# ToyotaResearchInstitute/idto

Measured on AMD Instinct MI355X. Metric: Gauss-Newton iters/sec (grad+Hessian+solve), mini_cheetah N=40, higher is better.
Workload: dtype f64; 1 GPU; mini_cheetah (nq=19, nv=18, 9 contact pairs), horizon N=40, dt=0.05, forward differences, one Gauss-Newton iteration per step; parallelism=single GPU

## Files before the change

### idto_amd/csrc/fd_kernel.h

```cpp
#pragma once

#include "arena_sizes.h"
#include "batch.h"
#include "id_eval.h"
#include "id_fast.h"

namespace idto_dev {

struct DevProblem {
  int N;
  double dt;
  const double* v_init;
  const double* q_nom;
  const double* v_nom;
  const double* Qq;
  const double* Qv;
  const double* R;
  const double* Qfq;
  const double* Qfv;
  const double* Qq0; const double* Qv0; const double* R0; const double* Qfq0; const double* Qfv0;
};

__host__ __device__ __forceinline__ DevProblem at_problem(DevProblem P, size_t o) {
  P.v_init = at_problem(P.v_init, o); P.q_nom = at_problem(P.q_nom, o); P.v_nom = at_problem(P.v_nom, o);
// ... 156 lines not shown
#pragma unroll
    for (int m = 0; m < NP; ++m) {
#pragma unroll
      for (int ur = 0; ur < TB; ++ur)
#pragma unroll
        for (int uc = 0; uc < TB; ++uc) {
          if (m == 0) acc[ur][uc] = a[m][ur].x * b[m][uc].x;
          else acc[ur][uc] = acc[ur][uc] + a[m][ur].x * b[m][uc].x;
          acc[ur][uc] = acc[ur][uc] + a[m][ur].y * b[m][uc].y;
        }
#pragma unroll
      for (int ur = 0; ur < TB; ++ur)
#pragma unroll
        for (int uc = 0; uc < TB; ++uc) asm volatile("" : "+v"(acc[ur][uc]));
      if (m == 0) FD_STAMP(18);
    }
    if (NV & 1) {
#pragma unroll
      for (int ur = 0; ur < TB; ++ur)
#pragma unroll
        for (int uc = 0; uc < TB; ++uc) acc[ur][uc] = acc[ur][uc] + A[ur][NV - 1] * B[uc][NV - 1];
    }
    FD_STAMP(19);
    return;
  }
  const int np = nv >> 1;
  double2 a[TB], b[TB];
#pragma unroll
  for (int u = 0; u < TB; ++u) {
    a[u] = reinterpret_cast<const double2*>(A[u])[0];
    b[u] = reinterpret_cast<const double2*>(B[u])[0];
  }
#pragma unroll
  for (int ur = 0; ur < TB; ++ur)
#pragma unroll
    for (int uc = 0; uc < TB; ++uc) {
      acc[ur][uc] = a[ur].x * b[uc].x;
      if (nv > 1) acc[ur][uc] = acc[ur][uc] + a[ur].y * b[uc].y;
    }
  FD_STAMP(18);
  double2 an[TB], bn[TB];
  if (np > 1) {
#pragma unroll
    for (int u = 0; u < TB; ++u) {
      an[u] = reinterpret_cast<const double2*>(A[u])[1];
      bn[u] = reinterpret_cast<const double2*>(B[u])[1];
    }
  }
  for (int m = 1; m < np; ++m) {
#pragma unroll
    for (int u = 0; u < TB; ++u) { a[u] = an[u]; b[u] = bn[u]; }
    const int mn = (m + 1 < np) ? m + 1 : m;
#pragma unroll
    for (int u = 0; u < TB; ++u) {
      an[u] = reinterpret_cast<const double2*>(A[u])[mn];
      bn[u] = reinterpret_cast<const double2*>(B[u])[mn];
    }
#pragma unroll
    for (int ur = 0; ur < TB; ++ur)
#pragma unroll
      for (int uc = 0; uc < TB; ++uc) {
        acc[ur][uc] = acc[ur][uc] + a[ur].x * b[uc].x;
        acc[ur][uc] = acc[ur][uc] + a[ur].y * b[uc].y;
      }
  }
  if ((nv & 1) && nv > 1) {
#pragma unroll
    for (int ur = 0; ur < TB; ++ur)
#pragma unroll
      for (int uc = 0; uc < TB; ++uc) acc[ur][uc] = acc[ur][uc] + A[ur][nv - 1] * B[uc][nv - 1];
  }
  FD_STAMP(19);
}


template <int SHAPE> struct FastShape {
  static constexpr TreeShape T = tree_shape(SHAPE);
  static constexpr int MAXC = T.MAXC, NP = T.NP, CJ = T.CJ, J0 = T.J0, K0 = T.K0, W2 = T.W2, GS = T.GS;
};
__host__ __device__ inline int fd_xch_doubles(int nxb, int threads, int npaths, int nstem = 0) {
  return (threads / npaths) * xch_eval_doubles(nxb, nstem);
}

template <int MAXC, int SHAPE = 0>
IDTO_DEV void fd_body(const DevModel& M, const DevContact& cp, const DevProblem& P, const double* __restrict__ q,
                      double* __restrict__ slab, int slab_stride, double* __restrict__ v_out,
                      double* __restrict__ a_out, double* __restrict__ nplus_out, const int k, int mode,
                      int stop_after, int echunk, double* __restrict__ terms) {
  extern __shared__ double lds[];
  constexpr bool FAST = SHAPE != 0 && SHAPE != SHAPE_XCH && SHAPE != SHAPE_STEM;
  const int tid = threadIdx.x, nt = blockDim.x;
  if (stop_after == 10) return;
#ifdef IDTO_FD_STAMPS
  long long st_arr[IDTO_FD_NSTAMPS] = {};
  long long* idto_fd_st = (tid == 0 || tid == IDTO_FD_STAMP_TID) ? st_arr : nullptr;
#endif
  FD_STAMP(0);
  const int nq = M.nq, nv = M.nv, K = M.npaths;
  const int bsz = nv * nq;
  const double dt = P.dt;

  const bool central = mode >= 2;
  const int NM = (mode == 2) ? 2 : ((mode == 3) ? 4 : 1);
  const int nP = (mode >= 1) ? NM * nq : 0;
  const int nT = (mode >= 1) ? NM * nq : 0;
  const int nM = (mode == 1) ? nv : (central ? NM * nq : 0);
  const int E = 1 + nP + nT + nM;

  double* qm1 = lds;
  double* q0 = qm1 + nq;
  double* q1 = q0 + nq;
  double* N0 = q1 + nq;
  double* N1 = N0 + bsz;
  double* v0 = N1 + bsz;
  double* v1 = v0 + nv;
  double* a0 = v1 + nv;
  double* edq = a0 + nv;
  const int EC = (echunk < E) ? echunk : E;
  double* edv = edq + E;
  double* eda = edv + E;
  double* etau = eda + E;
  double* eq = etau + E * nv;
  double* ev = eq + EC * nq;
  double* ea = ev + EC * nv;
  double* edump = ea + EC * nv;
  double* mblob = edump + nv;
  const int blob_lo = FAST ? M.fast_lo : 0, blob_n = FAST ? M.fast_n : M.blob_n;
  int* colinfo = reinterpret_cast<int*>(mblob + blob_n + (blob_n & 1));
  const int nvp = (nv + 1) & ~1, psz = nvp * nq;
  double* rec = reinterpret_cast<double*>(colinfo + nq + (nq & 1));
  rec += (rec - lds) & 1;
  double* xch = rec + (terms ? 6 * psz + 2 * nvp : 0);

  const bool sparse = M.nfloat == 0 || (M.nfloat > 0 && nt >= 128);
  const int ql = tid & 63, qcfg = tid >> 6;
  const bool quat_lane = sparse && M.nfloat > 0 && qcfg < 2 && ql >= 48 && ql < 60;
  double qf0[4];
  {
    const double* qq = q + (size_t)(k + (qcfg & 1)) * nq + (M.nfloat > 0 ? M.float_qs[0] : 0);
#pragma unroll
    for (int i = 0; i < 4; ++i) qf0[i] = qq[i];
  }
  double* wr = rec + 6 * psz;
  double* tw = wr + nvp;
  constexpr int BU = 8;
  double breg[BU];
#pragma unroll
  for (int u = 0; u < BU; ++u) {
    const int i = tid + u * nt;
    breg[u] = (i < blob_n) ? M.blob[blob_lo + i] : 0.0;
  }
  const bool qrow = tid < nq;
  const double g_qm1 = (qrow && k > 0) ? q[(k - 1) * nq + tid] : 0.0;
  const double g_q0 = qrow ? q[k * nq + tid] : 0.0, g_q1 = qrow ? q[(k + 1) * nq + tid] : 0.0;
  const double g_wr = (terms && mode != 0 && tid < nv) ? P.R[tid * nv + tid] : 0.0;
  const double g_nc0 = (sparse && tid < bsz) ? M.nplus_const[tid] : 0.0;
  const double g_nc1 = (sparse && tid + nt < bsz) ? M.nplus_const[tid + nt] : 0.0;
  const int g_ci = (sparse && qrow) ? M.colinfo[tid] : 0;
  const int rowinfo_r = (sparse && tid < nv) ? M.rowinfo[tid] : 0;
  asm volatile("" : "+v"(qf0[0]), "+v"(qf0[1]), "+v"(qf0[2]), "+v"(qf0[3]));
#pragma unroll
  for (int u = 0; u < BU; ++u) {
    const int i = tid + u * nt;
    if (i < blob_n) mblob[i] = breg[u];
  }
  for (int i = tid + BU * nt; i < blob_n; i += nt) mblob[i] = M.blob[blob_lo + i];
  if (qrow) { qm1[tid] = g_qm1; q0[tid] = g_q0; q1[tid] = g_q1; }
  for (int i = tid + nt; i < nq; i += nt) {
    qm1[i] = (k > 0) ? q[(k - 1) * nq + i] : 0.0;
    q0[i] = q[k * nq + i];
    q1[i] = q[(k + 1) * nq + i];
  }
  if (terms && mode != 0) {
    if (tid < nv) wr[tid] = g_wr;
    for (int l = tid + nt; l < nv; l += nt) wr[l] = P.R[l * nv + l];
  }
  if (sparse) {
    if (tid < bsz && g_nc0 == g_nc0) { N0[tid] = g_nc0; N1[tid] = g_nc0; }
    if (tid + nt < bsz && g_nc1 == g_nc1) { N0[tid + nt] = g_nc1; N1[tid + nt] = g_nc1; }
    for (int i = tid + 2 * nt; i < bsz; i += nt) {
      const double cst = M.nplus_const[i];
      if (cst == cst) { N0[i] = cst; N1[i] = cst; }
    }
    if (qrow) colinfo[tid] = g_ci;
    for (int i = tid + nt; i < nq; i += nt) colinfo[i] = M.colinfo[i];
    if (quat_lane) {
      const int e = ql - 48, r = e >> 2, c = e & 3;
      double* Nout = qcfg ? N1 : N0;
      for (int f = 0; f < M.nfloat; ++f) {
        const int qs = M.float_qs[f], vs = M.float_vs[f];
        double qq[4];
#pragma unroll
        for (int i = 0; i < 4; ++i) qq[i] = (f == 0) ? qf0[i] : q[(size_t)(k + qcfg) * nq + qs + i];
        const double nrm = __builtin_sqrt(((qq[0] * qq[0] + qq[1] * qq[1]) + qq[2] * qq[2]) + qq[3] * qq[3]);
        const double t0 = qq[0] / nrm, t1 = qq[1] / nrm, t2 = qq[2] / nrm, t3 = qq[3] / nrm;
        const double w2 = 2.0 * t0, x2 = 2.0 * t1, y2 = 2.0 * t2, z2 = 2.0 * t3;
        const double l0 = (r == 0) ? -x2 : ((r == 1) ? -y2 : -z2);
        const double l1 = (r == 0) ? w2 : ((r == 1) ? z2 : -y2);
        const double l2 = (r == 0) ? -z2 : ((r == 1) ? w2 : x2);
        const double l3 = (r == 0) ? y2 : ((r == 1) ? -x2 : w2);
        const double tc = (c == 0) ? t0 : ((c == 1) ? t1 : ((c == 2) ? t2 : t3));
        const double d0 = ((c == 0 ? 1.0 : 0.0) - t0 * tc) / nrm;
        const double d1 = ((c == 1 ? 1.0 : 0.0) - t1 * tc) / nrm;
        const double d2 = ((c == 2 ? 1.0 : 0.0) - t2 * tc) / nrm;
        const double d3 = ((c == 3 ? 1.0 : 0.0) - t3 * tc) / nrm;
        double acc = l0 * d0;
        acc += l1 * d1;
        acc += l2 * d2;
        acc += l3 * d3;
        Nout[(qs + c) * nv + vs + r] = acc;
      }
    }
  } else {
    for (int i = tid; i < bsz; i += nt) { N0[i] = 0.0; N1[i] = 0.0; }
  }
  FD_STAMP(1);
  __syncthreads();
  FD_STAMP(2);
  if (stop_after == 8) return;
  const DevModel Ml = rebase_model(M, mblob - blob_lo);
  if (!sparse) {
    for (int b = tid; b < Ml.nb; b += nt) {
      const int qs = Ml.qstart[b], vs = Ml.vstart[b], jt = Ml.jtype[b];
      if (jt == IDTO_JOINT_REVOLUTE || jt == IDTO_JOINT_PRISMATIC) colinfo[qs] = vs | 1 << 16;
      else if (jt == IDTO_JOINT_PLANAR) { for (int kq = 0; kq < 3; ++kq) colinfo[qs + kq] = (vs + kq) | 1 << 16; }
      else {
        for (int kq = 0; kq < 4; ++kq) colinfo[qs + kq] = vs | 3 << 16;
        for (int kq = 0; kq < 3; ++kq) colinfo[qs + 4 + kq] = (vs + 3 + kq) | 1 << 16;
      }
    }
    nplus_pair(Ml, q0, N0, q1, N1, tid, nt, true);
  }
  if (stop_after == 9) return;
  for (int r = tid; r < nv; r += nt) {
    double vr0, vr1;
    if (sparse) {
      const int ri = (r == tid) ? rowinfo_r : M.rowinfo[r];
      const int c0 = ri & 0xffff, c1 = c0 + (ri >> 16);
      double acc0 = N0[c0 * nv + r] * (q0[c0] - qm1[c0]), acc1 = N1[c0 * nv + r] * (q1[c0] - q0[c0]);
      for (int c = c0 + 1; c < c1; ++c) {
        acc0 += N0[c * nv + r] * (q0[c] - qm1[c]);
        acc1 += N1[c * nv + r] * (q1[c] - q0[c]);
      }
      vr0 = (k > 0) ? acc0 / dt : P.v_init[r];
      vr1 = acc1 / dt;
    } else {
      vr0 = (k > 0) ? velocity_row(Ml, N0, q0, qm1, dt, r) : P.v_init[r];
      vr1 = velocity_row(Ml, N1, q1, q0, dt, r);
    }
    v0[r] = vr0;
    v1[r] = vr1;
    a0[r] = (vr1 - vr0) / dt;
  }
  const double eps = 1.4901161193847656e-08;
  for (int e = (nt > 64) ? (tid + nt - 64) % nt : tid; e < E; e += nt) {
    double dq = 1.0;
    if (e >= 1 && (e < 1 + nP + nT || central)) {
      const int i = (e - 1) % nq;
      const double qi = (e < 1 + nP) ? q1[i] : ((e < 1 + nP + nT) ? q0[i] : qm1[i]);
      dq = eps * __builtin_fmax(1.0, __builtin_fabs(qi));
      const double temp = qi + dq;
      dq = temp - qi;
    }
    edq[e] = dq;
    const double dv = dq / dt;
    edv[e] = dv;
    eda[e] = dv / dt;
  }
  __syncthreads();

  auto trajectory_outputs = [&](int t0, int ts) {
    for (int r = t0; r < nv; r += ts) {
      v_out[(k + 1) * nv + r] = v1[r];
      a_out[k * nv + r] = a0[r];
      if (k == 0) v_out[r] = v0[r];
    }
    for (int i = t0; i < bsz; i += ts) {
      nplus_out[(size_t)(k + 1) * bsz + i] = N1[i];
      if (k == 0) nplus_out[i] = N0[i];
    }
  };
  const bool late_outputs = FAST && !central && stop_after != 1;
  if (!late_outputs) trajectory_outputs(tid, nt);

  FD_STAMP(3);
  if (stop_after == 1) return;
  const bool own_inputs = FAST && !central;
  for (int c0 = 0; c0 < E; c0 += (own_inputs ? E : EC)) {
  const int ce = own_inputs ? E : ((E - c0 < EC) ? E - c0 : EC);
  if (!own_inputs) {
  for (int idx = tid; idx < ce * nq; idx += nt) {
    const int el = idx / nq, c = idx - el * nq, e = c0 + el;
    double val = q1[c];
    if (e >= 1 && e < 1 + nP && c == (e - 1) % nq) {
      if (!central) {
        val = q1[c] + edq[e];
      } else {
        const int mi = (e - 1) / nq;
        const double mult = (mi == 0) ? 1.0 : ((mi == 1) ? -1.0 : ((mi == 2) ? 2.0 : -2.0));
        val = q1[c] + mult * edq[e];
      }
    }
    eq[idx] = val;
  }
  for (int idx = tid; idx < ce * nv; idx += nt) {
    const int el = idx / nv, j = idx - el * nv, e = c0 + el;
    double vv = v1[j], aa = a0[j];
    if (central && e >= 1) {
      const int g = (e - 1) / (NM * nq), mi = ((e - 1) / nq) % NM, i = (e - 1) % nq;
      const double mult = (mi == 0) ? 1.0 : ((mi == 1) ? -1.0 : ((mi == 2) ? 2.0 : -2.0));
      const double dv = edv[e], da = eda[e];
      const double n1 = N1[i * nv + j], n0 = N0[i * nv + j];
      if (g == 0) {
        vv = v1[j] + (mult * dv) * n1;
        aa = a0[j] + (mult * da) * n1;
      } else if (g == 1) {
        vv = v1[j] - (mult * dv) * n1;
        aa = a0[j] - (mult * da) * (n1 + n0);
      } else {
        aa = a0[j] + (mult * da) * n0;
      }
    } else if (e >= 1 && e < 1 + nP) {
      const int i = e - 1;
      const double dv = edv[e], da = eda[e];
      const double n1 = N1[i * nv + j];
      vv = v1[j] + dv * n1;
      aa = a0[j] + da * n1;
    } else if (e >= 1 + nP && e < 1 + nP + nT) {
      const int i = e - 1 - nP;
      const double dv = edv[e], da = eda[e];
      const double n1 = N1[i * nv + j], n0 = N0[i * nv + j];
      vv = v1[j] - dv * n1;
      aa = a0[j] - da * (n1 + n0);
    } else if (e >= 1 + nP + nT) {
      vv = 0.0;
      aa = (j == e - 1 - nP - nT) ? 1.0 : 0.0;
    }
    ev[idx] = vv;
    ea[idx] = aa;
  }
  __syncthreads();
  }

  if (stop_after == 2) return;
  const int groups = nt / K;
  if constexpr (FAST) {
    using FS = FastShape<SHAPE>;
    FastTab FT;
    FT.body = Ml.f_body; FT.cbody = Ml.f_cbody; FT.pairs = Ml.f_pairs; FT.seg = Ml.f_seg; FT.maxpp = Ml.f_maxpp;
    FT.gslots = Ml.gslots; FT.gcommon = Ml.gcommon;
    const int grp = tid / FS::NP, path = tid % FS::NP;
    for (int e0 = 0; e0 < ce; e0 += groups) {
      const int el = (e0 == 0) ? grp : e0 + (groups - 1 - grp);
      if (el < ce) {
        const bool full = central || c0 + el < 1 + nP + nT;
        if (own_inputs) {
          InFwd in;
          in.q1 = q1; in.v1 = v1; in.a0 = a0; in.N1 = N1; in.N0 = N0; in.nv = nv;
          in.kind = (el == 0) ? 0 : ((el < 1 + nP) ? 1 : ((el < 1 + nP + nT) ? 2 : 3));
          in.col = (el == 0) ? 0 : ((el < 1 + nP) ? el - 1 : ((el < 1 + nP + nT) ? el - 1 - nP : el - 1 - nP - nT));
          in.dq = edq[el];
          in.sdv = (in.kind == 2) ? -edv[el] : ((in.kind == 1) ? edv[el] : 0.0);
          in.sda = (in.kind == 2) ? -eda[el] : ((in.kind == 1) ? eda[el] : 0.0);
          in.keep = (in.kind == 3) ? 0ull : ~0ull;
          in.keep0 = (in.kind == 2) ? ~0ull : 0ull;
          id_eval_fast<FS::MAXC, FS::NP, FS::CJ, FS::J0, FS::K0, FS::W2, FS::GS>(FT, Ml.gravity, cp, path, full, in, etau + el * nv
#ifdef IDTO_FD_STAMPS
                                                                 , (e0 == 0) ? idto_fd_st : nullptr
#endif
          );
        } else {
          InLds in;
          in.q = eq + el * nq; in.v = ev + el * nv; in.a = ea + el * nv;
          id_eval_fast<FS::MAXC, FS::NP, FS::CJ, FS::J0, FS::K0, FS::W2, FS::GS>(FT, Ml.gravity, cp, path, full, in, etau + (c0 + el) * nv);
        }
      }
    }
    if (late_outputs && tid >= nt - 64) trajectory_outputs(tid - (nt - 64), 64);
  } else {
  for (int e0 = 0; e0 < ce; e0 += groups) {
    const int el = e0 + tid / K;
    const int path = tid % K;
    const int ee = (el < ce) ? el : 0;
    const bool full = central || c0 + ee < 1 + nP + nT;
    double* tau_dst = (el < ce) ? etau + (c0 + ee) * nv : edump;
    if constexpr (SHAPE == SHAPE_STEM)
      id_eval<MAXC, true, true>(Ml, cp, path, full, eq + ee * nq, ev + ee * nv, ea + ee * nv, tau_dst,
                                xch + (tid / K) * xch_eval_doubles(Ml.nxb, Ml.nstem));
    else if constexpr (SHAPE == SHAPE_XCH)
      id_eval<MAXC, true>(Ml, cp, path, full, eq + ee * nq, ev + ee * nv, ea + ee * nv, tau_dst, xch + (tid / K) * Ml.nxb * XREC);
    else
      id_eval<MAXC>(Ml, cp, path, full, eq + ee * nq, ev + ee * nv, ea + ee * nv, tau_dst);
  }
  }
  __syncthreads();
  }

  FD_STAMP(12);
  if (stop_after == 3) return;
  constexpr bool GROWS = FAST;
  constexpr bool CSIZES = FAST && SHAPE <= kNumSizedShapes;
  constexpr int CNQ = CSIZES ? tree_shape_nq(SHAPE) : 0, CNV = CSIZES ? tree_shape_nv(SHAPE) : 0, CNVP = (CNV + 1) & ~1;
  const int tnq = CNQ ? CNQ : nq, tnv = CNQ ? CNV : nv, tbsz = CNQ ? CNV * CNQ : bsz, tnvp = CNQ ? CNVP : nvp, tpsz = CNQ ? CNVP * CNQ : psz;
  double* sl = slab + (size_t)k * slab_stride;
  double* Mk = sl;
  double* Tk = sl + tbsz;
  double* Pk = sl + 2 * tbsz;
  double* tauk = sl + 3 * tbsz;
  for (int r = tid; r < tnv; r += nt) tauk[r] = etau[r];
  if constexpr (GROWS)
    if (terms && mode != 0)
      for (int r = nt - 1 - tid; r < tnvp; r += nt) tw[r] = (r < tnv) ? etau[r] * wr[r] : 0.0;
  if (mode == 1) {
    const double sc = 1 / dt / dt;
    const double* Mcols = etau + (1 + tnq + tnq) * tnv;
    const double fillM = (k == 0) ? __builtin_nan("") : 0.0;
    constexpr int RU = 2;
    for (int base = tid; base < tbsz; base += RU * nt) {
      int ii[RU], rr[RU], j0[RU], cnt[RU];
      bool ok[RU];
      double tp[RU], tt[RU], t0[RU], dqp[RU], dqt[RU], w[RU], mc[RU][3], n0[RU][3];
#pragma unroll
      for (int u = 0; u < RU; ++u) {
        const int idx = base + u * nt;
        ok[u] = idx < tbsz;
        const int id = ok[u] ? idx : 0;
        ii[u] = id / tnv; rr[u] = id - ii[u] * tnv;
        const int ci = colinfo[ii[u]];
        j0[u] = ci & 0xffff; cnt[u] = ci >> 16;
        tp[u] = etau[(1 + ii[u]) * tnv + rr[u]]; tt[u] = etau[(1 + tnq + ii[u]) * tnv + rr[u]]; t0[u] = etau[rr[u]];
        dqp[u] = edq[1 + ii[u]]; dqt[u] = edq[1 + tnq + ii[u]];
        w[u] = terms ? wr[rr[u]] : 0.0;
#pragma unroll
        for (int t = 0; t < 3; ++t) {
          const int j = (t < cnt[u]) ? j0[u] + t : j0[u];
          mc[u][t] = Mcols[j * tnv + rr[u]];
          n0[u][t] = N0[ii[u] * tnv + j];
        }
      }
      FD_STAMP(13);
      double pvs[RU], tvs[RU], accs[RU];
#pragma unroll
      for (int u = 0; u < RU; ++u) {
        if (!ok[u]) continue;
        pvs[u] = (tp[u] - t0[u]) / dqp[u];
        tvs[u] = (k >= 1) ? (tt[u] - t0[u]) / dqt[u] : 0.0;
        double acc = (sc * mc[u][0]) * n0[u][0];
        if (cnt[u] > 1) acc += (sc * mc[u][1]) * n0[u][1];
        if (cnt[u] > 2) acc += (sc * mc[u][2]) * n0[u][2];
// ... 56 lines not shown
  const float inb = 1.0f / (float)nb;
  for (int tile = tid; tile < ntiles; tile += nt) {
    if (stop_after == 6 && tile >= 3 * ntt) break;
    int xa, sb, tr, tc, ob;
    const bool lower = tile < 3 * ntt;
    if (lower) {
      const int which = (tile >= ntt) + (tile >= 2 * ntt);
      int rem = tile - which * ntt;
      tc = 0;
      if constexpr (CNQ != 0) {
        constexpr int NB = (CNQ + TB - 1) / TB, NBR = CNQ / TB + 1;
        int off = 0;
#pragma unroll
        for (int t = 0, S = 0; t < NB - 1; ++t) {
          S += NBR - t;
          const bool ge = rem >= S;
          tc += ge; off = ge ? S : off;
        }
        rem -= off;
      } else {
        while (rem >= nbr - tc) { rem -= nbr - tc; ++tc; }
      }
      tr = tc + rem;
      xa = which; sb = which; ob = which * qq;
    } else {
      const int it = tile - 3 * ntt, which = (it >= nbb) + (it >= 2 * nbb), e = it - which * nbb;
      if constexpr (CNQ != 0) tc = e / nb;
      else tc = (int)(((float)e + 0.5f) * inb);
      tr = e - tc * nb;
      xa = (which == 1) ? 1 : 0; sb = (which == 0) ? 1 : 2; ob = (3 + which) * qq;
    }
    const double* A[TB];
    const double* B[TB];
#pragma unroll
    for (int u = 0; u < TB; ++u) {
      const int r = tr * TB + u, c = tc * TB + u;
      if constexpr (GROWS) A[u] = r < tnq ? rec + (3 + xa) * tpsz + r * tnvp : tw;
      else A[u] = rec + (3 + xa) * tpsz + (r < tnq ? r : tnq - 1) * tnvp;
      B[u] = rec + sb * tpsz + (c < tnq ? c : tnq - 1) * tnvp;
    }
    double acc[TB][TB];
    FD_STAMP(17);
#ifdef IDTO_FD_STAMPS
    asm_dot_tile<TB, CNV>(A, B, tnv, acc, idto_fd_st);
#else
    asm_dot_tile<TB, CNV>(A, B, tnv, acc);
#endif
#pragma unroll
    for (int ur = 0; ur < TB; ++ur)
#pragma unroll
      for (int uc = 0; uc < TB; ++uc) {
        const int r = tr * TB + ur, c = tc * TB + uc;
        if (r < tnq && c < tnq && (!lower || r >= c)) stage[ob + c * tnq + r] = acc[ur][uc];
        if constexpr (GROWS)
          if (lower && r == tnq && c < tnq && stop_after != 7) stage[6 * qq + xa * tnq + c] = acc[ur][uc];
      }
    FD_STAMP(20);
  }
  FD_STAMP(21);
  if constexpr (!GROWS)
    if (stop_after != 7)
      for (int it = nt - 1 - tid; it < 3 * tnq; it += nt) {
        const int which = (it >= tnq) + (it >= 2 * tnq), j = it - which * tnq;
        const double* J = rec + which * tpsz + j * tnvp;
        double acc = (etau[0] * wr[0]) * J[0];
        for (int r = 1; r < tnv; ++r) acc += (etau[r] * wr[r]) * J[r];
        stage[6 * qq + which * tnq + j] = acc;
      }
  FD_STAMP(22);
#ifdef IDTO_FD_STAMPS
  if (idto_fd_st && k == 1 && 2 * IDTO_FD_NSTAMPS <= tbsz)
    for (int i = 0; i < IDTO_FD_NSTAMPS; ++i)
      nplus_out[(size_t)(k + 1) * tbsz + (tid == 0 ? 0 : IDTO_FD_NSTAMPS) + i] = (double)(st_arr[i] - st_arr[0]);
#endif
}

template <int MAXC, int SHAPE = 0>
__global__ void __launch_bounds__(256) fd_kernel(DevModel M, DevContact cp, DevProblem P, const double* __restrict__ q,
                          double* __restrict__ slab, int slab_stride, double* __restrict__ v_out,
                          double* __restrict__ a_out, double* __restrict__ nplus_out, int k_begin, int mode,
                          int stop_after, int echunk, size_t pstride, double* __restrict__ terms, AltSel alt) {
  const size_t o = (size_t)blockIdx.y * pstride;
  const size_t w = o + (size_t)alt_offset(alt, o);
  fd_body<MAXC, SHAPE>(M, cp, at_problem(P, o), at_problem(q, o), at_problem(slab, w), slab_stride, at_problem(v_out, w),
                       at_problem(a_out, w), at_problem(nplus_out, w), k_begin + (int)blockIdx.x, mode, stop_after, echunk,
                       terms ? at_problem(terms, w) : nullptr);
}

template <int MAXC, int SHAPE = 0>
__global__ void __launch_bounds__(256) fd_along_kernel(DevModel M, DevContact cp, DevProblem P, const double* __restrict__ q,
                          double* __restrict__ slab, int slab_stride, double* __restrict__ v_out,
                          double* __restrict__ a_out, double* __restrict__ nplus_out, int k_begin, int stop_after,
                          int echunk, size_t cstride, const double* __restrict__ gate) {
  if (gate && *gate != 0.0) return;
  const size_t w = (size_t)blockIdx.y * cstride;
  fd_body<MAXC, SHAPE>(M, cp, P, at_problem(q, w), at_problem(slab, w), slab_stride, at_problem(v_out, w),
                       at_problem(a_out, w), at_problem(nplus_out, w), k_begin + (int)blockIdx.x, 0, stop_after, echunk, nullptr);
}

template <int MAXC, int SHAPE = 0>
__global__ void __launch_bounds__(256) fd_along_batch_kernel(DevModel M, DevContact cp, DevProblem P, const double* __restrict__ q,
                          double* __restrict__ slab, int slab_stride, double* __restrict__ v_out,
                          double* __restrict__ a_out, double* __restrict__ nplus_out, int k_begin, int stop_after,
                          int echunk, size_t cstride, const double* __restrict__ gate, size_t pstride, size_t bstride,
                          size_t gstride) {
  if (gate && *at_problem(gate, (size_t)blockIdx.z * gstride) != 0.0) return;
  const size_t w = (size_t)blockIdx.z * bstride + (size_t)blockIdx.y * cstride;
  fd_body<MAXC, SHAPE>(M, cp, at_problem(P, (size_t)blockIdx.z * pstride), at_problem(q, w), at_problem(slab, w), slab_stride,
                       at_problem(v_out, w), at_problem(a_out, w), at_problem(nplus_out, w), k_begin + (int)blockIdx.x, 0,
                       stop_after, echunk, nullptr);
}

template <int MAXC, int SHAPE = 0>
__global__ void __launch_bounds__(256) fd_models_kernel(const double* __restrict__ records, size_t mstride, size_t cat, size_t mat,
                          DevProblem P, const double* __restrict__ q, double* __restrict__ slab, int slab_stride,
                          double* __restrict__ v_out, double* __restrict__ a_out, double* __restrict__ nplus_out, int k_begin,
                          int mode, int stop_after, int echunk, size_t pstride, double* __restrict__ terms, AltSel alt) {
  const size_t o = (size_t)blockIdx.y * pstride;
  const size_t w = o + (size_t)alt_offset(alt, o);
  const RecordPtr rec = record_at(records, (size_t)blockIdx.y * mstride);
  fd_body<MAXC, SHAPE>(*(const DevModel*)(rec + mat), *(const DevContact*)(rec + cat), at_problem(P, o), at_problem(q, o),
                       at_problem(slab, w), slab_stride, at_problem(v_out, w), at_problem(a_out, w), at_problem(nplus_out, w),
                       k_begin + (int)blockIdx.x, mode, stop_after, echunk, terms ? at_problem(terms, w) : nullptr);
}

template <int MAXC, int SHAPE = 0>
__global__ void __launch_bounds__(256) fd_along_models_kernel(const double* __restrict__ records, size_t mstride, size_t cat,
                          size_t mat, DevProblem P, const double* __restrict__ q, double* __restrict__ slab, int slab_stride,
                          double* __restrict__ v_out, double* __restrict__ a_out, double* __restrict__ nplus_out, int k_begin,
                          int stop_after, int echunk, size_t cstride, const double* __restrict__ gate, size_t pstride,
                          size_t bstride, size_t gstride) {
  if (gate && *at_problem(gate, (size_t)blockIdx.z * gstride) != 0.0) return;
  const size_t w = (size_t)blockIdx.z * bstride + (size_t)blockIdx.y * cstride;
  const RecordPtr rec = record_at(records, (size_t)blockIdx.z * mstride);
  fd_body<MAXC, SHAPE>(*(const DevModel*)(rec + mat), *(const DevContact*)(rec + cat), at_problem(P, (size_t)blockIdx.z * pstride),
                       at_problem(q, w), at_problem(slab, w), slab_stride, at_problem(v_out, w), at_problem(a_out, w),
                       at_problem(nplus_out, w), k_begin + (int)blockIdx.x, 0, stop_after, echunk, nullptr);
}

}
```

### idto_amd/csrc/id_fast.h

```cpp
#pragma once

#include "id_eval.h"

#ifdef IDTO_FD_STAMPS
#ifndef IDTO_FD_STAMP_TID
#define IDTO_FD_STAMP_TID 192
#endif
#define IDTO_FD_NSTAMPS 24
#define FD_STAMP(i) do { __builtin_amdgcn_sched_barrier(0); asm volatile("" ::: "memory"); if (idto_fd_st) idto_fd_st[i] = (long long)__builtin_readcyclecounter(); asm volatile("" ::: "memory"); __builtin_amdgcn_sched_barrier(0); } while (0)
#else
#define FD_STAMP(i) do { } while (0)
#endif

namespace idto_dev {

template <int CTRL>
IDTO_DEV double quad_perm(double x) {
  int lo = __double2loint(x), hi = __double2hiint(x);
  lo = __builtin_amdgcn_update_dpp(0, lo, CTRL, 0xf, 0xf, true);
  hi = __builtin_amdgcn_update_dpp(0, hi, CTRL, 0xf, 0xf, true);
  return __hiloint2double(hi, lo);
}
template <int NP>
IDTO_DEV V3 tree_sum_fast(V3 v) {
// ... 150 lines not shown
  const double exponent = -phi / cp.sigma;
  if (exponent >= 37) compliant_fn = -cp.k * phi;
  else compliant_fn = cp.sigma * cp.k * idto::detmath::log(1 + idto::detmath::exp(exponent));
  const double fn = compliant_fn * dissipation;
  const V3 that = (-vt) / __builtin_sqrt(cp.vs * cp.vs + dot(vt, vt));
  const V3 ft = (that * cp.mu) * fn;
  *fo = n1 * fn + ft;
  *fc = -*fo;
  *no = cross(pOC, *fo);
  *nc = cross(pCC, *fc);
  return true;
}

IDTO_DEV void inertial_wrench_rec(const double* rec, const M3& R, V3 w, V3 al, V3 a, V3 g, V3* f_in, V3* n_in) {
  const V3 cW = R * ldv3(rec + FB_COM);
  const V3 t1 = cross(al, cW);
  const V3 t2 = cross(w, cross(w, cW));
  const V3 acom = (a + t1) + t2;
  *f_in = (acom - g) * rec[FB_MASS];
  const V3 wB = tmul(R, w), alB = tmul(R, al);
  const double* I = rec + FB_INERTIA;
  const V3 Iw = mk(fma3(I[0], wB.x, I[3], wB.y, I[4], wB.z), fma3(I[3], wB.x, I[1], wB.y, I[5], wB.z),
                   fma3(I[4], wB.x, I[5], wB.y, I[2], wB.z));
  const V3 Ial = mk(fma3(I[0], alB.x, I[3], alB.y, I[4], alB.z), fma3(I[3], alB.x, I[1], alB.y, I[5], alB.z),
                    fma3(I[4], alB.x, I[5], alB.y, I[2], alB.z));
  const V3 nB = Ial + cross(wB, Iw);
  *n_in = R * nB + cross(cW, *f_in);
}

template <bool HAS_COMMON>
IDTO_DEV void pair_group(const double* plist, int segword, const DevContact& cp, const BodyState& C, const BodyState& cb,
                         V3* fext, V3* next, V3* cfe, V3* cne) {
  const int start = segword & 0xffff, count = segword >> 16;
  for (int j = start; j < start + count; ++j) {
    const double* pr = plist + j * FP_STRIDE;
    V3 fc, nc, fo, no;
    if (pair_eval<HAS_COMMON>(pr, cp, C, cb, &fc, &nc, &fo, &no)) {
      *fext = *fext + fc; *next = *next + nc;
      if (HAS_COMMON) {
        const bool oc = reinterpret_cast<const int*>(pr + FP_INFO)[3] != 0;
        if (oc) { *cfe = *cfe + fo; *cne = *cne + no; }
      }
    }
  }
}

struct FastTab {
  const double* body;
  const double* cbody;
  const double* pairs;
  const int* seg;
  int maxpp;
  unsigned long long gslots;
  int gcommon;
};

struct InLds {
  const double *q, *v, *a;
  IDTO_DEV double Q(int i) const { return q[i]; }
  IDTO_DEV double V(int j) const { return v[j]; }
  IDTO_DEV double A(int j) const { return a[j]; }
  IDTO_DEV InLds laundered() const { InLds o = *this; o.v = lds_launder(v); return o; }
};
struct InFwd {
  const double *q1, *v1, *a0, *N1, *N0;
  int nv, kind, col;
  double dq, sdv, sda;
  unsigned long long keep, keep0;
  IDTO_DEV static double and_bits(double x, unsigned long long m) {
    return __longlong_as_double((long long)((unsigned long long)__double_as_longlong(x) & m));
  }
  IDTO_DEV double Q(int i) const {
    const double x = q1[i], xp = x + dq;
    return (kind == 1 && i == col) ? xp : x;
  }
  IDTO_DEV double V(int j) const { return and_bits(v1[j], keep) + sdv * N1[col * nv + j]; }
  IDTO_DEV double A(int j) const {
    const double unit = (kind == 3 && j == col) ? 1.0 : 0.0;
    return (and_bits(a0[j], keep) + unit) + sda * (N1[col * nv + j] + and_bits(N0[col * nv + j], keep0));
  }
  IDTO_DEV InFwd laundered() const { InFwd o = *this; o.v1 = lds_launder(v1); o.N1 = lds_launder(N1); return o; }
};

template <int MAXC, int NP, int CJ, int J0, int K0, int W2, int GS = 0, class In>
IDTO_DEV void id_eval_fast(const FastTab& T, const double* gravity, const DevContact& cp, int path, bool full,
                           const In& in_fwd, double* tau, long long* idto_fd_st = nullptr) {
  const In& in = in_fwd;
  constexpr bool HAS_COMMON = (CJ == IDTO_JOINT_FLOATING);
  const V3 zero = mk(0, 0, 0);
  const V3 g = full ? mk(gravity[0], gravity[1], gravity[2]) : zero;
  const double* bt = T.body + (size_t)path * (MAXC * FB_STRIDE);
  const double* ct = T.cbody;
  const double* plist = T.pairs + (size_t)path * (T.maxpp * FP_STRIDE);
  const int* seg = T.seg + path * (MAXC + 2);

  int qs[MAXC], vs[MAXC];
#pragma unroll
  for (int s = 0; s < MAXC; ++s) {
    const int2 ix = *reinterpret_cast<const int2*>(bt + s * FB_STRIDE + FB_IDX);
    qs[s] = ix.x; vs[s] = ix.y;
  }
  int cqs = 0, cvs = 0;
  if (HAS_COMMON) {
    const int2 ix = *reinterpret_cast<const int2*>(ct + FB_IDX);
    cqs = ix.x; cvs = ix.y;
  }
  double qj[MAXC], vj[MAXC], aj[MAXC];
  double q0x = 0, q0y = 0, v0x = 0, v0y = 0, a0x = 0, a0y = 0;
#pragma unroll
  for (int s = 0; s < MAXC; ++s) {
    if (s == 0 && J0 == IDTO_JOINT_PLANAR) {
      q0x = in.Q(qs[0]); q0y = in.Q(qs[0] + 1); qj[0] = in.Q(qs[0] + 2);
      v0x = in.V(vs[0]); v0y = in.V(vs[0] + 1); vj[0] = in.V(vs[0] + 2);
      a0x = in.A(vs[0]); a0y = in.A(vs[0] + 1); aj[0] = in.A(vs[0] + 2);
    } else {
      qj[s] = in.Q(qs[s]); vj[s] = in.V(vs[s]); aj[s] = in.A(vs[s]);
    }
  }
  double cq[7], cv[6], ca[6];
  if (HAS_COMMON) {
#pragma unroll
    for (int i = 0; i < 7; ++i) cq[i] = in.Q(cqs + i);
#pragma unroll
    for (int i = 0; i < 6; ++i) { cv[i] = in.V(cvs + i); ca[i] = in.A(cvs + i); }
  }
  FD_STAMP(4);
  double sn[MAXC], cs[MAXC];
#pragma unroll
  for (int s = 0; s < MAXC; ++s) idto::detmath::sincos(qj[s], &sn[s], &cs[s]);
  FD_STAMP(5);

  double rc_next[FB_PREFETCH];
  prefetch_record(bt, rc_next);
  BodyState cb;
  cb.R = ident3(); cb.p = zero; cb.w = zero; cb.v = zero;
  V3 cb_al = zero, cb_a = zero, cb_fin = zero, cb_nin = zero;
  V3 cfe = zero, cne = zero;
  if (HAS_COMMON) {
    const M3 R_WF = ldm3(ct + FB_XPF);
    const V3 d1 = ldv3(ct + FB_XPF + 9);
    const M3 R_FM = quat_to_rot(cq);
    const V3 d2 = R_WF * mk(cq[4], cq[5], cq[6]);
    const V3 w_rel = R_WF * mk(cv[0], cv[1], cv[2]);
    const V3 v_rel = R_WF * mk(cv[3], cv[4], cv[5]);
    const V3 al_rel = R_WF * mk(ca[0], ca[1], ca[2]);
    const V3 a_rel = R_WF * mk(ca[3], ca[4], ca[5]);
    cb.R = R_WF * R_FM;
    cb.p = zero + (d1 + d2);
    cb.w = zero + w_rel;
    cb.v = zero + v_rel;
    cb_al = zero + al_rel;
    cb_a = zero + a_rel;
    inertial_wrench_rec(ct, cb.R, cb.w, cb_al, cb_a, GS ? body_gravity(T.gcommon != 0, g) : g, &cb_fin, &cb_nin);
    pin(cb_fin); pin(cb_nin);
    if (full) pair_group<false>(plist, seg[0], cp, cb, cb, &cfe, &cne, &cfe, &cne);
  }

  FD_STAMP(6);
  V3 r[MAXC], hW[MAXC], ft[MAXC], nt[MAXC];
  BodyState bs_prev;
  bs_prev.R = ident3(); bs_prev.p = zero; bs_prev.w = zero; bs_prev.v = zero;
  ParentKin P;
  P.R = ident3(); P.p = zero; P.w = zero; P.v = zero; P.al = zero; P.a = zero;
#pragma unroll
  for (int s = 0; s < MAXC; ++s) {
    double rec[FB_PREFETCH];
#pragma unroll
    for (int i = 0; i < FB_PREFETCH; ++i) rec[i] = rc_next[i];
    const bool world = (s == 0 && K0 == PK_WORLD) || (W2 >= 1 && s == W2);
    if (s == 0 && K0 == PK_COMMON) { P.R = cb.R; P.p = cb.p; P.w = cb.w; P.v = cb.v; P.al = cb_al; P.a = cb_a; }
    const M3 R_WF = world ? ldm3(rec + FB_XPF) : P.R * ldm3(rec + FB_XPF);
    const V3 d1 = world ? ldv3(rec + FB_XPF + 9) : P.R * ldv3(rec + FB_XPF + 9);
    BodyState bs;
    V3 al, acc;
    if (s == 0 && J0 == IDTO_JOINT_PLANAR) {
      M3 R_FM = ident3();
      R_FM.m[0] = cs[0]; R_FM.m[1] = -sn[0]; R_FM.m[3] = sn[0]; R_FM.m[4] = cs[0];
      const V3 ex = col(R_WF, 0), ey = col(R_WF, 1), ez = col(R_WF, 2);
      const V3 d2 = ex * q0x + ey * q0y;
      const V3 v_rel = ex * v0x + ey * v0y;
      const V3 a_rel = ex * a0x + ey * a0y;
      const V3 w_rel = ez * vj[0];
      const V3 al_rel = ez * aj[0];
      hW[0] = zero;
      bs.R = R_WF * R_FM;
      r[0] = d1 + d2;
      bs.p = zero + r[0];
      bs.w = zero + w_rel;
      bs.v = zero + v_rel;
      al = zero + al_rel;
      acc = zero + a_rel;
    } else {
      const V3 axis = ldv3(rec + FB_AXIS);
      const M3 R_FM = axis_angle(axis, sn[s], cs[s]);
      hW[s] = R_WF * axis;
      const V3 w_rel = hW[s] * vj[s];
      const V3 al_rel = hW[s] * aj[s];
      bs.R = R_WF * R_FM;
      r[s] = d1 + zero;
      if (world) {
        bs.p = zero + r[s];
        bs.w = zero + w_rel;
        bs.v = zero;
        al = zero + al_rel;
        acc = zero;
      } else {
        bs.p = P.p + r[s];
        bs.w = P.w + w_rel;
        bs.v = (P.v + cross(P.w, r[s])) + zero;
        al = (P.al + al_rel) + cross(P.w, w_rel);
        acc = ((P.a + cross(P.al, r[s])) + cross(P.w, cross(P.w, r[s]))) + zero;
      }
    }
    V3 fin, nin;
    inertial_wrench_rec(rec, bs.R, bs.w, al, acc, GS ? body_gravity(slot_gravity(T.gslots, path, s), g) : g, &fin, &nin);
    pin(fin); pin(nin); pin(r[s]); pin(hW[s]);
    if (s == MAXC - 1) FD_STAMP(8);
    if (s + 1 < MAXC) prefetch_record(bt + (s + 1) * FB_STRIDE, rc_next);
    V3 fext = zero, next = zero;
    if (W2 >= 1 && s == W2) {
      V3 ofe = zero, one = zero;
      if (full) pair_group<true>(plist, seg[1 + s], cp, bs, bs_prev, &fext, &next, &ofe, &one);
      ft[W2 - 1] = ft[W2 - 1] - ofe;
      nt[W2 - 1] = nt[W2 - 1] - one;
      pin(ft[W2 - 1]); pin(nt[W2 - 1]);
    } else if (full) {
      pair_group<HAS_COMMON>(plist, seg[1 + s], cp, bs, cb, &fext, &next, &cfe, &cne);
    }
    ft[s] = fin - fext;
    nt[s] = nin - next;
    pin(ft[s]); pin(nt[s]);
    if (W2 >= 1 && s == W2 - 1) bs_prev = bs;
    P.R = bs.R; P.p = bs.p; P.w = bs.w; P.v = bs.v; P.al = al; P.a = acc;
    if (s == 0) FD_STAMP(7);
    if (s == MAXC - 1) FD_STAMP(9);
  }
  if (HAS_COMMON && full) pair_group<false>(plist, seg[MAXC + 1], cp, cb, cb, &cfe, &cne, &cfe, &cne);

  FD_STAMP(10);
  const In inb = in_fwd.laundered();
  const double* btb = lds_launder(bt);
  V3 child_f = zero, child_n = zero;
  V3 root_f = zero, root_n = zero;
#pragma unroll
  for (int s = MAXC - 1; s >= 0; --s) {
    const double* rec = btb + s * FB_STRIDE;
    V3 f = ft[s], n = nt[s];
    if (s + 1 < MAXC && s + 1 != W2) { f = f + child_f; n = n + child_n; }
    if (s == 0 && J0 == IDTO_JOINT_PLANAR) {
      const M3 R_WF = ldm3(rec + FB_XPF);
      const double t0 = dot(col(R_WF, 0), f), t1 = dot(col(R_WF, 1), f), t2 = dot(col(R_WF, 2), n);
      tau[vs[0]] = full ? t0 + rec[FB_DAMP] * inb.V(vs[0]) : t0;
      tau[vs[0] + 1] = full ? t1 + rec[FB_DAMP + 1] * inb.V(vs[0] + 1) : t1;
      tau[vs[0] + 2] = full ? t2 + rec[FB_DAMP + 2] * inb.V(vs[0] + 2) : t2;
    } else {
      const double t = dot(hW[s], n);
      tau[vs[s]] = full ? t + rec[FB_DAMP] * inb.V(vs[s]) : t;
    }
    const V3 cf = f, cn = n + cross(r[s], f);
    if (s > 0) { child_f = cf; child_n = cn; }
    else if (K0 == PK_COMMON) { root_f = cf; root_n = cn; }
  }

  FD_STAMP(11);
  if (HAS_COMMON) {
    const V3 ext_f = tree_sum_fast<NP>(cfe);
    const V3 ext_n = tree_sum_fast<NP>(cne);
    const V3 ch_f = tree_sum_fast<NP>(root_f);
    const V3 ch_n = tree_sum_fast<NP>(root_n);
    const V3 f = (cb_fin - ext_f) + ch_f;
    const V3 n = (cb_nin - ext_n) + ch_n;
    if (path == 0) {
      const double* ctb = lds_launder(ct);
      const M3 R_WF = ldm3(ctb + FB_XPF);
      const V3 nF = tmul(R_WF, n), fF = tmul(R_WF, f);
      const double t6[6] = {nF.x, nF.y, nF.z, fF.x, fF.y, fF.z};
#pragma unroll
      for (int i = 0; i < 6; ++i) tau[cvs + i] = full ? t6[i] + ctb[FB_DAMP + i] * inb.V(cvs + i) : t6[i];
    }
  }
}

}
```

Baseline: 13250 GN iters/s.

## Precompute fast-ID front (indices, sincos) before barrier and reassign quaternion N+ to chain wave

Adds an AHEAD mode to the FD kernel. Non-chain waves compute the front part of the fast inverse dynamics (joint indices, configuration reads, sincos) for their first perturbation before the __syncthreads, so that work overlaps the velocity/acceleration setup. The last wave alone does the quaternion N+ entries and the v/a rows, using wave-level fences instead of a block barrier. Epsilon assignment is moved onto the remaining threads. This adds register pressure and more complex thread-role logic in exchange for shorter serialized latency per block.

```diff
diff --git a/idto_amd/csrc/fd_kernel.h b/idto_amd/csrc/fd_kernel.h
--- a/idto_amd/csrc/fd_kernel.h
+++ b/idto_amd/csrc/fd_kernel.h
@@ -262,7 +262,27 @@
   return (threads / npaths) * xch_eval_doubles(nxb, nstem);
 }
 
-template <int MAXC, int SHAPE = 0>
+IDTO_DEV double nplus_quat_entry(const double (&qq)[4], const int r, const int c) {
+  const double nrm = __builtin_sqrt(((qq[0] * qq[0] + qq[1] * qq[1]) + qq[2] * qq[2]) + qq[3] * qq[3]);
+  const double t0 = qq[0] / nrm, t1 = qq[1] / nrm, t2 = qq[2] / nrm, t3 = qq[3] / nrm;
+  const double w2 = 2.0 * t0, x2 = 2.0 * t1, y2 = 2.0 * t2, z2 = 2.0 * t3;
+  const double l0 = (r == 0) ? -x2 : ((r == 1) ? -y2 : -z2);
+  const double l1 = (r == 0) ? w2 : ((r == 1) ? z2 : -y2);
+  const double l2 = (r == 0) ? -z2 : ((r == 1) ? w2 : x2);
+  const double l3 = (r == 0) ? y2 : ((r == 1) ? -x2 : w2);
+  const double tc = (c == 0) ? t0 : ((c == 1) ? t1 : ((c == 2) ? t2 : t3));
+  const double d0 = ((c == 0 ? 1.0 : 0.0) - t0 * tc) / nrm;
+  const double d1 = ((c == 1 ? 1.0 : 0.0) - t1 * tc) / nrm;
+  const double d2 = ((c == 2 ? 1.0 : 0.0) - t2 * tc) / nrm;
+  const double d3 = ((c == 3 ? 1.0 : 0.0) - t3 * tc) / nrm;
+  double acc = l0 * d0;
+  acc += l1 * d1;
+  acc += l2 * d2;
+  acc += l3 * d3;
+  return acc;
+}
+
+template <int MAXC, int SHAPE = 0, bool AHEAD = false>
 IDTO_DEV void fd_body(const DevModel& M, const DevContact& cp, const DevProblem& P, const double* __restrict__ q,
                       double* __restrict__ slab, int slab_stride, double* __restrict__ v_out,
                       double* __restrict__ a_out, double* __restrict__ nplus_out, const int k, int mode,
@@ -314,10 +334,21 @@
 
   const bool sparse = M.nfloat == 0 || (M.nfloat > 0 && nt >= 128);
   const int ql = tid & 63, qcfg = tid >> 6;
-  const bool quat_lane = sparse && M.nfloat > 0 && qcfg < 2 && ql >= 48 && ql < 60;
+  constexpr bool FRONT = AHEAD && FAST && SHAPE <= kNumSizedShapes && tree_shape(FAST ? SHAPE : 1).CJ == IDTO_JOINT_FLOATING;
+  bool front = false, chain_wave = false;
+  int qsel = qcfg & 1, vrow = tid;
+  if constexpr (FRONT) {
+    front = mode == 1 && sparse && M.nfloat == 1 && stop_after != 1;
+    if (front) {
+      chain_wave = __builtin_amdgcn_readfirstlane(qcfg) == (nt >> 6) - 1;
+      qsel = (ql >= 12 && ql < 24) ? 1 : 0;
+      vrow = chain_wave ? ql : nv;
+    }
+  }
+  const bool quat_lane = sparse && M.nfloat > 0 && qcfg < 2 && ql >= 48 && ql < 60 && !front;
   double qf0[4];
   {
-    const double* qq = q + (size_t)(k + (qcfg & 1)) * nq + (M.nfloat > 0 ? M.float_qs[0] : 0);
+    const double* qq = q + (size_t)(k + qsel) * nq + (M.nfloat > 0 ? M.float_qs[0] : 0);
 #pragma unroll
     for (int i = 0; i < 4; ++i) qf0[i] = qq[i];
   }
@@ -337,7 +368,7 @@
   const double g_nc0 = (sparse && tid < bsz) ? M.nplus_const[tid] : 0.0;
   const double g_nc1 = (sparse && tid + nt < bsz) ? M.nplus_const[tid + nt] : 0.0;
   const int g_ci = (sparse && qrow) ? M.colinfo[tid] : 0;
-  const int rowinfo_r = (sparse && tid < nv) ? M.rowinfo[tid] : 0;
+  const int rowinfo_r = (sparse && vrow < nv) ? M.rowinfo[vrow] : 0;
   asm volatile("" : "+v"(qf0[0]), "+v"(qf0[1]), "+v"(qf0[2]), "+v"(qf0[3]));
 #pragma unroll
   for (int u = 0; u < BU; ++u) {
@@ -372,23 +403,7 @@
         double qq[4];
 #pragma unroll
         for (int i = 0; i < 4; ++i) qq[i] = (f == 0) ? qf0[i] : q[(size_t)(k + qcfg) * nq + qs + i];
-        const double nrm = __builtin_sqrt(((qq[0] * qq[0] + qq[1] * qq[1]) + qq[2] * qq[2]) + qq[3] * qq[3]);
-        const double t0 = qq[0] / nrm, t1 = qq[1] / nrm, t2 = qq[2] / nrm, t3 = qq[3] / nrm;
-        const double w2 = 2.0 * t0, x2 = 2.0 * t1, y2 = 2.0 * t2, z2 = 2.0 * t3;
-        const double l0 = (r == 0) ? -x2 : ((r == 1) ? -y2 : -z2);
-        const double l1 = (r == 0) ? w2 : ((r == 1) ? z2 : -y2);
-        const double l2 = (r == 0) ? -z2 : ((r == 1) ? w2 : x2);
-        const double l3 = (r == 0) ? y2 : ((r == 1) ? -x2 : w2);
-        const double tc = (c == 0) ? t0 : ((c == 1) ? t1 : ((c == 2) ? t2 : t3));
-        const double d0 = ((c == 0 ? 1.0 : 0.0) - t0 * tc) / nrm;
-        const double d1 = ((c == 1 ? 1.0 : 0.0) - t1 * tc) / nrm;
-        const double d2 = ((c == 2 ? 1.0 : 0.0) - t2 * tc) / nrm;
-        const double d3 = ((c == 3 ? 1.0 : 0.0) - t3 * tc) / nrm;
-        double acc = l0 * d0;
-        acc += l1 * d1;
-        acc += l2 * d2;
-        acc += l3 * d3;
-        Nout[(qs + c) * nv + vs + r] = acc;
+        Nout[(qs + c) * nv + vs + r] = nplus_quat_entry(qq, r, c);
       }
     }
   } else {
@@ -412,10 +427,20 @@
     nplus_pair(Ml, q0, N0, q1, N1, tid, nt, true);
   }
   if (stop_after == 9) return;
-  for (int r = tid; r < nv; r += nt) {
+  if constexpr (FRONT)
+    if (chain_wave) {
+      if (ql < 24) {
+        const int e = (ql < 12) ? ql : ql - 12, r = e >> 2, c = e & 3;
+        (qsel ? N1 : N0)[(M.float_qs[0] + c) * nv + M.float_vs[0] + r] = nplus_quat_entry(qf0, r, c);
+      }
+      __builtin_amdgcn_fence(__ATOMIC_RELEASE, "wavefront");
+      __builtin_amdgcn_wave_barrier();
+      __builtin_amdgcn_fence(__ATOMIC_ACQUIRE, "wavefront");
+    }
+  for (int r = vrow; r < nv; r += (front ? 64 : nt)) {
     double vr0, vr1;
     if (sparse) {
-      const int ri = (r == tid) ? rowinfo_r : M.rowinfo[r];
+      const int ri = (r == vrow) ? rowinfo_r : M.rowinfo[r];
       const int c0 = ri & 0xffff, c1 = c0 + (ri >> 16);
       double acc0 = N0[c0 * nv + r] * (q0[c0] - qm1[c0]), acc1 = N1[c0 * nv + r] * (q1[c0] - q0[c0]);
       for (int c = c0 + 1; c < c1; ++c) {
@@ -433,7 +458,8 @@
     a0[r] = (vr1 - vr0) / dt;
   }
   const double eps = 1.4901161193847656e-08;
-  for (int e = (nt > 64) ? (tid + nt - 64) % nt : tid; e < E; e += nt) {
+  const int elo = (front && nt >= 192) ? 64 : 0, ew = (front && nt > 64) ? nt - 64 - elo : nt;
+  for (int e = front ? ((tid >= elo && tid < elo + ew) ? tid - elo : E) : ((nt > 64) ? (tid + nt - 64) % nt : tid); e < E; e += ew) {
     double dq = 1.0;
     if (e >= 1 && (e < 1 + nP + nT || central)) {
       const int i = (e - 1) % nq;
@@ -447,6 +473,27 @@
     edv[e] = dv;
     eda[e] = dv / dt;
   }
+  using FS = FastShape<FAST ? SHAPE : 1>;
+  FastFront<FS::MAXC> pre;
+  const bool formed = front && !chain_wave;
+  if constexpr (FRONT)
+    if (formed) {
+      const int el = tid / FS::NP;
+      if (el < E) {
+        FastTab FT;
+        FT.body = Ml.f_body; FT.cbody = Ml.f_cbody;
+        InFwd in;
+        in.q1 = q1; in.v1 = v1; in.a0 = a0; in.N1 = N1; in.N0 = N0; in.nv = nv;
+        in.kind = (el >= 1 && el < 1 + nP) ? 1 : 0;
+        in.col = (in.kind == 1) ? el - 1 : 0;
+        const double qi = q1[in.col];
+        double dq = eps * __builtin_fmax(1.0, __builtin_fabs(qi));
+        const double temp = qi + dq;
+        in.dq = temp - qi;
+        id_fast_front<FS::MAXC, FS::CJ, FS::J0>(FT, tid % FS::NP, in, pre);
+      }
+      FD_STAMP(23);
+    }
   __syncthreads();
 
   auto trajectory_outputs = [&](int t0, int ts) {
@@ -525,7 +572,6 @@
   if (stop_after == 2) return;
   const int groups = nt / K;
   if constexpr (FAST) {
-    using FS = FastShape<SHAPE>;
     FastTab FT;
     FT.body = Ml.f_body; FT.cbody = Ml.f_cbody; FT.pairs = Ml.f_pairs; FT.seg = Ml.f_seg; FT.maxpp = Ml.f_maxpp;
     FT.gslots = Ml.gslots; FT.gcommon = Ml.gcommon;
@@ -540,11 +586,14 @@
           in.kind = (el == 0) ? 0 : ((el < 1 + nP) ? 1 : ((el < 1 + nP + nT) ? 2 : 3));
           in.col = (el == 0) ? 0 : ((el < 1 + nP) ? el - 1 : ((el < 1 + nP + nT) ? el - 1 - nP : el - 1 - nP - nT));
           in.dq = edq[el];
+          if constexpr (FRONT)
+            if (!(formed && e0 == 0)) id_fast_front<FS::MAXC, FS::CJ, FS::J0>(FT, path, in, pre);
           in.sdv = (in.kind == 2) ? -edv[el] : ((in.kind == 1) ? edv[el] : 0.0);
           in.sda = (in.kind == 2) ? -eda[el] : ((in.kind == 1) ? eda[el] : 0.0);
           in.keep = (in.kind == 3) ? 0ull : ~0ull;
           in.keep0 = (in.kind == 2) ? ~0ull : 0ull;
-          id_eval_fast<FS::MAXC, FS::NP, FS::CJ, FS::J0, FS::K0, FS::W2, FS::GS>(FT, Ml.gravity, cp, path, full, in, etau + el * nv
+          id_eval_fast<FS::MAXC, FS::NP, FS::CJ, FS::J0, FS::K0, FS::W2, FS::GS>(FT, Ml.gravity, cp, path, full, in, pre,
+                                                                 FRONT, etau + el * nv
 #ifdef IDTO_FD_STAMPS
                                                                  , (e0 == 0) ? idto_fd_st : nullptr
 #endif
@@ -767,9 +816,9 @@
                           int stop_after, int echunk, size_t pstride, double* __restrict__ terms, AltSel alt) {
   const size_t o = (size_t)blockIdx.y * pstride;
   const size_t w = o + (size_t)alt_offset(alt, o);
-  fd_body<MAXC, SHAPE>(M, cp, at_problem(P, o), at_problem(q, o), at_problem(slab, w), slab_stride, at_problem(v_out, w),
-                       at_problem(a_out, w), at_problem(nplus_out, w), k_begin + (int)blockIdx.x, mode, stop_after, echunk,
-                       terms ? at_problem(terms, w) : nullptr);
+  fd_body<MAXC, SHAPE, true>(M, cp, at_problem(P, o), at_problem(q, o), at_problem(slab, w), slab_stride, at_problem(v_out, w),
+                             at_problem(a_out, w), at_problem(nplus_out, w), k_begin + (int)blockIdx.x, mode, stop_after, echunk,
+                             terms ? at_problem(terms, w) : nullptr);
 }
 
 template <int MAXC, int SHAPE = 0>
diff --git a/idto_amd/csrc/id_fast.h b/idto_amd/csrc/id_fast.h
--- a/idto_amd/csrc/id_fast.h
+++ b/idto_amd/csrc/id_fast.h
@@ -256,9 +256,54 @@
   IDTO_DEV InFwd laundered() const { InFwd o = *this; o.v1 = lds_launder(v1); o.N1 = lds_launder(N1); return o; }
 };
 
+template <int MAXC>
+struct FastFront {
+  int qs[MAXC], vs[MAXC], cqs, cvs;
+  double q0x, q0y, cq[7], sn[MAXC], cs[MAXC];
+};
+template <int MAXC, int CJ, int J0, class In>
+IDTO_DEV void id_fast_front(const FastTab& T, int path, const In& in, FastFront<MAXC>& F) {
+  constexpr bool HAS_COMMON = (CJ == IDTO_JOINT_FLOATING);
+  const double* bt = T.body + (size_t)path * (MAXC * FB_STRIDE);
+  const double* ct = T.cbody;
+#pragma unroll
+  for (int s = 0; s < MAXC; ++s) {
+    const int2 ix = *reinterpret_cast<const int2*>(bt + s * FB_STRIDE + FB_IDX);
+    F.qs[s] = ix.x; F.vs[s] = ix.y;
+  }
+  F.cqs = 0; F.cvs = 0;
+  if (HAS_COMMON) {
+    const int2 ix = *reinterpret_cast<const int2*>(ct + FB_IDX);
+    F.cqs = ix.x; F.cvs = ix.y;
+  }
+  double qj[MAXC];
+  F.q0x = 0; F.q0y = 0;
+#pragma unroll
+  for (int s = 0; s < MAXC; ++s) {
+    if (s == 0 && J0 == IDTO_JOINT_PLANAR) {
+      F.q0x = in.Q(F.qs[0]); F.q0y = in.Q(F.qs[0] + 1); qj[0] = in.Q(F.qs[0] + 2);
+    } else {
+      qj[s] = in.Q(F.qs[s]);
+    }
+  }
+#pragma unroll
+  for (int i = 0; i < 7; ++i) F.cq[i] = HAS_COMMON ? in.Q(F.cqs + i) : 0.0;
+#pragma unroll
+  for (int s = 0; s < MAXC; ++s) idto::detmath::sincos(qj[s], &F.sn[s], &F.cs[s]);
+#pragma unroll
+  for (int s = 0; s < MAXC; ++s) asm volatile("" : "+v"(F.qs[s]), "+v"(F.vs[s]), "+v"(F.sn[s]), "+v"(F.cs[s]));
+  if (HAS_COMMON) {
+    asm volatile("" : "+v"(F.cqs), "+v"(F.cvs));
+#pragma unroll
+    for (int i = 0; i < 7; ++i) asm volatile("" : "+v"(F.cq[i]));
+  }
+  if (J0 == IDTO_JOINT_PLANAR) asm volatile("" : "+v"(F.q0x), "+v"(F.q0y));
+}
+
 template <int MAXC, int NP, int CJ, int J0, int K0, int W2, int GS = 0, class In>
 IDTO_DEV void id_eval_fast(const FastTab& T, const double* gravity, const DevContact& cp, int path, bool full,
-                           const In& in_fwd, double* tau, long long* idto_fd_st = nullptr) {
+                           const In& in_fwd, const FastFront<MAXC>& pre, bool have_pre, double* tau,
+                           long long* idto_fd_st = nullptr) {
   const In& in = in_fwd;
   constexpr bool HAS_COMMON = (CJ == IDTO_JOINT_FLOATING);
   const V3 zero = mk(0, 0, 0);
@@ -269,18 +314,42 @@
   const int* seg = T.seg + path * (MAXC + 2);
 
   int qs[MAXC], vs[MAXC];
+  int cqs = 0, cvs = 0;
+  double qj[MAXC], vj[MAXC], aj[MAXC];
+  double q0x = 0, q0y = 0, v0x = 0, v0y = 0, a0x = 0, a0y = 0;
+  double cq[7], cv[6], ca[6];
+  double sn[MAXC], cs[MAXC];
+  if (have_pre) {
+#pragma unroll
+    for (int s = 0; s < MAXC; ++s) { qs[s] = pre.qs[s]; vs[s] = pre.vs[s]; sn[s] = pre.sn[s]; cs[s] = pre.cs[s]; }
+    cqs = pre.cqs; cvs = pre.cvs; q0x = pre.q0x; q0y = pre.q0y;
+#pragma unroll
+    for (int i = 0; i < 7; ++i) cq[i] = pre.cq[i];
+#pragma unroll
+    for (int s = 0; s < MAXC; ++s) {
+      if (s == 0 && J0 == IDTO_JOINT_PLANAR) {
+        v0x = in.V(vs[0]); v0y = in.V(vs[0] + 1); vj[0] = in.V(vs[0] + 2);
+        a0x = in.A(vs[0]); a0y = in.A(vs[0] + 1); aj[0] = in.A(vs[0] + 2);
+      } else {
+        vj[s] = in.V(vs[s]); aj[s] = in.A(vs[s]);
+      }
+    }
+    if (HAS_COMMON) {
+#pragma unroll
+      for (int i = 0; i < 6; ++i) { cv[i] = in.V(cvs + i); ca[i] = in.A(cvs + i); }
+    }
+    FD_STAMP(4);
+    FD_STAMP(5);
+  } else {
 #pragma unroll
   for (int s = 0; s < MAXC; ++s) {
     const int2 ix = *reinterpret_cast<const int2*>(bt + s * FB_STRIDE + FB_IDX);
     qs[s] = ix.x; vs[s] = ix.y;
   }
-  int cqs = 0, cvs = 0;
   if (HAS_COMMON) {
     const int2 ix = *reinterpret_cast<const int2*>(ct + FB_IDX);
     cqs = ix.x; cvs = ix.y;
   }
-  double qj[MAXC], vj[MAXC], aj[MAXC];
-  double q0x = 0, q0y = 0, v0x = 0, v0y = 0, a0x = 0, a0y = 0;
 #pragma unroll
   for (int s = 0; s < MAXC; ++s) {
     if (s == 0 && J0 == IDTO_JOINT_PLANAR) {
@@ -291,7 +360,6 @@
       qj[s] = in.Q(qs[s]); vj[s] = in.V(vs[s]); aj[s] = in.A(vs[s]);
     }
   }
-  double cq[7], cv[6], ca[6];
   if (HAS_COMMON) {
 #pragma unroll
     for (int i = 0; i < 7; ++i) cq[i] = in.Q(cqs + i);
@@ -299,10 +367,10 @@
     for (int i = 0; i < 6; ++i) { cv[i] = in.V(cvs + i); ca[i] = in.A(cvs + i); }
   }
   FD_STAMP(4);
-  double sn[MAXC], cs[MAXC];
 #pragma unroll
   for (int s = 0; s < MAXC; ++s) idto::detmath::sincos(qj[s], &sn[s], &cs[s]);
   FD_STAMP(5);
+  }
 
   double rc_next[FB_PREFETCH];
   prefetch_record(bt, rc_next);
@@ -454,5 +522,11 @@
     }
   }
 }
-
-}
+template <int MAXC, int NP, int CJ, int J0, int K0, int W2, int GS = 0, class In>
+IDTO_DEV void id_eval_fast(const FastTab& T, const double* gravity, const DevContact& cp, int path, bool full,
+                           const In& in_fwd, double* tau, long long* idto_fd_st = nullptr) {
+  FastFront<MAXC> none;
+  id_eval_fast<MAXC, NP, CJ, J0, K0, W2, GS>(T, gravity, cp, path, full, in_fwd, none, false, tau, idto_fd_st);
+}
+
+}
```

Result: no change. 13250 GN iters/s, median of 2 (+0.0%).
